# tmkhang1999/TextMAE-Image-Compression

Hardware: AMD Instinct MI355X
Metric: images/sec encode+decode+rate, ViT-B 256×256 batch64, 1/2/4/8 MI355X (higher is better)
Workload: dtype bf16; 1 GPU; MCM forward eval: ids+ViT-B/16 enc (K=144 of 256 patches) + LIC hyperprior + EB/GC rates + ViT dec 512/8/16 + unpatchify; img_size=256, num_keep_patches=144, per_gpu_batch=64, global_batch=64, parallelism=replicas x1, hip_graph=True

## Files before the change

### include/tmae.h

```cpp
#ifndef TMAE_H
#define TMAE_H

#include <stdint.h>

#ifdef __cplusplus
extern "C" {
#endif

#define TMAE_ABI_VERSION 1

enum { TMAE_OK = 0, TMAE_EINVAL = 1, TMAE_EHIP = 2 };
enum { TMAE_F32 = 0, TMAE_BF16 = 1 };
enum { TMAE_ACT_NONE = 0, TMAE_ACT_GELU = 1, TMAE_ACT_RELU = 2  };

const char* tmae_last_error_string(void);
int tmae_abi_version(void);

int tmae_ids_shuffle(const float* scores, int64_t* ids_shuffle, int64_t* ids_restore, int n, int L, int K,
                     int sum_lanes, void* stream);


int tmae_layernorm_fwd(const float* x, const float* gamma, const float* beta, void* y, int rows, int D,
                       int row_group, int group_stride, int row_offset, float eps, int out_dtype, void* stream);

// ... 245 lines not shown
                 int dh, float scale, int dtype, void* stream);
int tmae_patch_gather(const float* imgs, const int64_t* ids_shuffle, void* out, int n, int C, int H, int W, int patch,
                      int L, int keep, int dtype, void* stream);

typedef struct tmae_wgrad_args {
  const void* a; int lda; int a_G, a_Gs, a_off;
  const void* b; int ldb; int b_G, b_Gs, b_off;
  int b_conv; const void* b2; int b_c1, b_ld2, b_H, b_W, b_stride, b_Cin;
  int M, N, K;
  float* work; long long work_elems;
  float* out; long long o_base, o_sm, o_sc, o_st; int o_cp; int accumulate;
  float* bias_out; int bias_accumulate;
  int slot_div;
  int nb; long long s_a, s_b, s_b2, s_out, s_bias;
} tmae_wgrad_args;
int tmae_wgrad(const tmae_wgrad_args* args, int dtype, void* stream);
long long tmae_wgrad_workspace(int M, int N, int K, int dtype);
long long tmae_wgrad_workspace_nb(int M, int N, int K, int dtype, int slot_div, int nb);

int tmae_dgrad_linear(const void* dy, int ldy, int row_group, int group_stride, int row_offset, const void* wt, int M,
                      int N, int K, void* out, int out_f32, int ldo, const void* pre, int ldp, float* acc32, int ld32,
                      int dtype, void* stream);

typedef struct tmae_conv_dgrad_args {
  const void* dy; int ldy;
  int n, H, W, stride, cout, cin;
  const void* wd;
  void* out; int out_f32, ldo; const void* pre; int ldp;
  float* acc[3]; int ld_acc[3]; int lim[3];
  int nb; long long s_dy, s_wd, s_out, s_pre;
} tmae_conv_dgrad_args;
int tmae_conv_dgrad(const tmae_conv_dgrad_args* args, int dtype, void* stream);

int tmae_relayout(const float* src, void* dst, int dst_dtype, int d0, int d1, int d2, int d3, long long s0, long long s1,
                  long long s2, long long s3, void* stream);
int tmae_relayout_multi(const long long* table, int ntensors, long long nchunks, void* stream);

int tmae_colsum(const void* x, int x_dtype, int ld, int rows, int C, int row_group, int group_stride, int row_offset,
                float* work, long long work_elems, float* out, int accumulate, void* stream);

int tmae_layernorm_bwd(const float* x, const float* gamma, const float* dy, const float* dres, float* dx32, void* dxop,
                       int op_dtype, int rows, int D, int row_group, int group_stride, int row_offset, float eps,
                       float* work, long long work_elems, float* dgamma, float* dbeta, float* dres_colsum, int accumulate,
                       void* stream);

int tmae_unshuffle_bwd(const void* dy, int dy_f32, int ldy, const void* pre, int ldp, void* out, int n, int H, int W,
                       int C4, int dtype, void* stream);
int tmae_gelu_bwd(const void* dy, int dy_f32, const void* pre, void* out, long long total, int dtype, void* stream);
int tmae_lrp_bwd(const float* g32, int ld32, const float* g32b, int ld32b, const void* g16, int ld16, const float* t,
                 int ldt, void* dt, int lddt, float* gsum, int ldgs, int rows, int C, int dtype, void* stream);
int tmae_copy2d(const void* src, int lds, void* dst, int ldd, int rows, int cols, int esz, void* stream);
int tmae_gc_bwd(const float* y, int ldy, int yoff, const float* mu, const float* sigma, int ld_ms, const float* noise,
                int Mtot, const float* glik, const float* gyp, int ldg, float* dy, int lddy, void* dmu, void* dsigma,
                int ldd, int n, int HW, int sw, int dtype, void* stream);
int tmae_eb_bwd(const tmae_eb_params* params, const float* z, const float* noise, const float* glik,
                const float* gzhat, float* dz, int n, int C, int HW, const tmae_eb_params* grads, int accumulate,
                void* stream);
int tmae_eb_aux_bwd(const tmae_eb_params* params, const float* target, const float* gout, float* dquantiles, int C,
                    int accumulate, void* stream);
int tmae_bpp_bwd(const float* lik, const float* gout, float* dlik, long long n, double num_pixels, void* stream);
int tmae_patchify(const float* imgs, void* out, int n, int C, int H, int W, int patch, int dtype, void* stream);
int tmae_unpatchify(const float* tokens, float* imgs, int n, int C, int H, int W, int patch, void* stream);
int tmae_decoder_embed_bwd_gather(const float* dec_grad, const int64_t* ids_shuffle, void* tok_grad, int n, int ntok,
                                  int L, int D, int dtype, float* mask_part, float* dmask, int accumulate,
                                  void* stream);
int tmae_add(const float* a, const float* b, float* out, long long n, void* stream);

int tmae_adam(float* p, const float* g, float* m, float* v, long long n, float lr, float beta1, float beta2, float eps,
              float weight_decay, int step, const float* clip, void* stream);
int tmae_adam_multi(const long long* table, int ntensors, long long nchunks, float lr, float beta1, float beta2,
                    float eps, float weight_decay, const float* clip, void* stream);
int tmae_grad_norm(const float* g, long long n, double* work, float max_norm, float* out, void* stream);
int tmae_scale(float* g, long long n, const float* scale, void* stream);

int tmae_distortion_fwd(const float* x, const float* y, int P, int H, int W, float* hwork, float* dmaps, double* part,
                        float* out, void* stream);
int tmae_distortion_bwd(const float* x, const float* y, int P, int H, int W, const float* dmaps, float* vwork,
                        const float* gout, float* gx, void* stream);

int tmae_gemm_plan(int M, int N, int K, int batch, int dtype, char* out, int len);

int tmae_gemm_force_tile(int index);

int tmae_mha_plan(int T, int dh, int dtype, int backward, char* out, int len);

int tmae_mha_force_stream(int on);

#ifdef __cplusplus
}
#endif

#endif
```

### textmae-image-compression_amd/_lib.py

```python
from __future__ import annotations

import ctypes
import os

PKG_DIR = os.path.dirname(os.path.abspath(__file__))
LIB_PATH = os.environ.get("TMAE_LIB") or os.path.join(PKG_DIR, "lib", "libtmae.so")

TMAE_F32, TMAE_BF16 = 0, 1
ACT_NONE, ACT_GELU, ACT_RELU = 0, 1, 2

P, I, F = ctypes.c_void_p, ctypes.c_int, ctypes.c_float


LL = ctypes.c_longlong


class ConvArgs(ctypes.Structure):
    _fields_ = [
        ("x1", P), ("c1", I), ("ld1", I), ("x1_s1", LL), ("x1_s2", LL),
        ("x2", P), ("c2", I), ("ld2", I), ("x2_s1", LL), ("x2_s2", LL),
        ("n", I), ("H", I), ("W", I), ("stride", I),
        ("w", P), ("w_s1", LL), ("w_s2", LL),
        ("bias", P), ("b_s1", LL), ("b_s2", LL),
        ("cout", I), ("act", I), ("pixel_shuffle", I),
# ... 28 lines not shown
        ("wd", P),
        ("out", P), ("out_f32", I), ("ldo", I), ("pre", P), ("ldp", I),
        ("acc", P * 3), ("ld_acc", I * 3), ("lim", I * 3),
        ("nb", I), ("s_dy", LL), ("s_wd", LL), ("s_out", LL), ("s_pre", LL),
    ]


LSTK_MAXL = 5


class LicStackArgs(ctypes.Structure):
    _fields_ = [
        ("n", I), ("G", I), ("nb1", I), ("nb2", I), ("nlayers", I),
        ("x1", P), ("c1", I), ("ld1", I), ("x1_s", LL * 2),
        ("x2", P), ("c2", I), ("ld2", I), ("x2_s", LL * 2),
        ("w", P * LSTK_MAXL), ("w_s", (LL * 2) * LSTK_MAXL),
        ("bias", P * LSTK_MAXL), ("b_s", (LL * 2) * LSTK_MAXL),
        ("cout", I * LSTK_MAXL),
        ("addend", P), ("ld_add", I), ("a_s", LL * 2),
        ("y", P), ("y_f32", I), ("ldy", I), ("y_s", LL * 2),
        ("lrp_src", P), ("ld_src", I), ("src_s", LL * 2),
        ("y2", P), ("ldy2", I), ("y2_s", LL * 2),
        ("flags", I),
        ("cn", I), ("cw", P * LSTK_MAXL), ("cb", P * LSTK_MAXL), ("ccout", I * LSTK_MAXL),
        ("cx1", P), ("cc1", I), ("cld1", I),
        ("yv", P), ("ldyv", I),
        ("cadd", P), ("cld_add", I),
        ("csrc", P), ("cld_src", I),
        ("cy", P), ("cldy", I),
        ("cy2", P), ("cldy2", I),
        ("cs_x1", LL), ("cs_yv", LL), ("cs_src", LL), ("cs_add", LL), ("cs_y", LL), ("cs_y2", LL),
        ("cs_w", LL * LSTK_MAXL), ("cs_b", LL * LSTK_MAXL),
        ("sv_pre", P * LSTK_MAXL), ("sv_act", P * LSTK_MAXL), ("sv_s", (LL * 2) * LSTK_MAXL),
        ("sv_t", P), ("sv_t_s", LL * 2),
        ("csv_pre", P * LSTK_MAXL), ("csv_act", P * LSTK_MAXL), ("cs_sv", LL * LSTK_MAXL),
        ("csv_t", P), ("cs_t", LL),
        ("racc", P * 3), ("rld", I * 3), ("rlim", I * 3), ("rs", LL * 3),
    ]


class LicLatentArgs(ctypes.Structure):
    _fields_ = [
        ("n", I), ("G", I), ("cin", I), ("nb", I),
        ("x", P * 4), ("ldx", I),
        ("w", P), ("nfr", I), ("blk", LL),
        ("f_off", I * 4), ("f_lo", I), ("f_hi", I),
        ("y", P), ("ldy", I),
        ("y_s", LL * 4), ("bias", P * 4), ("act", I), ("y_bf16", I),
    ]


class EBParams(ctypes.Structure):
    _fields_ = [("matrix", ctypes.c_void_p * 5), ("bias", ctypes.c_void_p * 5), ("factor", ctypes.c_void_p * 4),
                ("quantiles", ctypes.c_void_p)]


SIGNATURES = {
    "tmae_abi_version": [],
    "tmae_ids_shuffle": [P, P, P, I, I, I, I, P],
    "tmae_layernorm_fwd": [P, P, P, P, I, I, I, I, I, F, I, P],
    "tmae_linear_fwd": [P, I, I, I, I, I, P, P, P, I, I, P, I, I, I, I, I, I, P],
    "tmae_linear_residual_fwd": [P, I, P, P, P, I, I, I, I, I, P],
    "tmae_patch_embed_fwd": [P, P, P, P, P, P, I, I, I, I, I, I, I, I, I, P],
    "tmae_patch_embed_gathered": [P, P, P, P, P, P, I, I, I, I, I, I, P],
    "tmae_cls_rows": [P, P, P, I, I, I, P],
    "tmae_mha_fwd": [P, P, I, I, I, I, F, I, P],
    "tmae_qkv_attn_fwd": [P, P, P, P, I, I, I, I, F, I, P],
    "tmae_decoder_embed_fwd": [P, I, P, P, P, P, P, I, I, I, I, I, I, P],
    "tmae_mask_rows": [P, P, P, P, I, I, I, I, P],
    "tmae_decoder_pred_fwd": [P, P, P, P, I, I, I, I, I, I, I, I, P],
    "tmae_decoder_pred_cp_fwd": [P, P, P, P, I, I, I, I, I, I, I, I, P],
    "tmae_conv3x3": [ctypes.POINTER(ConvArgs), I, P],
    "tmae_lic_stack": [ctypes.POINTER(LicStackArgs), P],
    "tmae_lic_latent": [ctypes.POINTER(LicLatentArgs), P],
    "tmae_gc_slices_fwd": [P, I, I, P, P, LL, I, P, P, I, P, I, I, P, I, I, I, I, I, P],
    "tmae_eb_likelihood_fwd": [P, ctypes.POINTER(EBParams), P, P, P, I, P, I, I, I, P],
    "tmae_eb_aux_loss": [ctypes.POINTER(EBParams), P, P, P, I, P],
    "tmae_gc_likelihood_fwd": [P, P, P, P, P, P, I, F, P],
    "tmae_nhwc_to_nchw": [P, I, P, I, I, I, P],
    "tmae_crop_normalize_u8": [P, I, I, I, P, I, I, ctypes.POINTER(F), ctypes.POINTER(F), P, P],
    "tmae_bpp_sum": [P, LL, P, LL, P, P, ctypes.c_double, P],
    "tmae_gemm_plan": [I, I, I, I, I, ctypes.c_char_p, I],
    "tmae_mha_plan": [I, I, I, I, ctypes.c_char_p, I],
    "tmae_mae_masking": [P, P, P, P, I, I, I, P],
    "tmae_mae_loss": [P, P, P, I, I, I, I, I, I, I, P, P, P],
    "tmae_mae_loss_bwd": [P, P, P, I, I, I, I, I, I, I, P, P, P, I, P],
    "tmae_gc_slices_code": [P, I, I, P, P, LL, I, P, I, P, I, I, P, I, I, I, I, I, P, P, P, I, P],
    "tmae_gc_indexes": [P, LL, I, I, I, I, I, P, I, F, P, P],
    "tmae_gc_dequantize": [P, P, LL, I, I, I, I, I, I, P, I, I, P, I, P],
    "tmae_gc_pmf": [P, P, I, I, P, P, P],
    "tmae_eb_pmf": [ctypes.POINTER(EBParams), P, P, I, I, P, P, P],
    "tmae_eb_symbols": [P, ctypes.POINTER(EBParams), P, I, I, I, P, P],
    "tmae_eb_dequantize": [P, ctypes.POINTER(EBParams), P, I, I, I, P, I, P],
    "tmae_invert_permutation": [P, P, I, I, P],
    "tmae_pmf_to_quantized_cdf": [P, I, I, P],
    "tmae_rans_encoder_create": [ctypes.POINTER(ctypes.c_void_p)],
    "tmae_rans_encode_with_indexes": [P, P, P, LL, P, I, P, P, I],
    "tmae_rans_encoder_flush": [P, ctypes.POINTER(ctypes.c_longlong)],
    "tmae_rans_encoder_take": [P, P, LL],
    "tmae_rans_encoder_destroy": [P],
    "tmae_rans_decoder_create": [P, LL, ctypes.POINTER(ctypes.c_void_p)],
    "tmae_rans_decode_with_indexes": [P, P, LL, P, I, P, P, I, P],
    "tmae_rans_decoder_destroy": [P],
    "tmae_rans_encode_streams": [P, LL, LL, P, LL, LL, I, I, I, P, I, P, P, I, P, LL, P, P, P],
    "tmae_rans_pack_streams": [P, LL, P, I, P, LL, P, P, P],
    "tmae_rans_decode_streams": [P, LL, P, P, P, LL, LL, P, LL, LL, I, I, I, I, P, I, P, P, I, P, P, P, I, P],
    "tmae_rans_encode_lanes": [P, LL, LL, P, LL, LL, I, I, I, P, I, P, P, I, P, LL, P, P, I, P],
    "tmae_rans_decode_lanes": [P, LL, P, P, P, LL, LL, P, LL, LL, I, I, I, I, P, I, P, P, I, P, P, P, I, I, P],
    "tmae_huffman_build": [P, LL, P, P, P, I, ctypes.POINTER(I)],
    "tmae_huffman_encode": [P, LL, P, P, P, I, P, LL, ctypes.POINTER(LL)],
    "tmae_huffman_decode": [ctypes.c_char_p, LL, P, P, P, I, P, LL, ctypes.POINTER(LL)],
    "tmae_image_metrics": [P, P, I, I, I, I, P, LL, P, P],
    "tmae_image_scores": [P, I, I, I, I, I, P, LL, P, P],
    "tmae_vgg_prep": [P, I, I, I, I, I, P, I, P],
    "tmae_vgg_prep_bwd": [P, I, I, I, I, I, P, I, P],
    "tmae_maxpool2": [P, I, I, I, I, P, P, I, P],
    "tmae_maxpool2_bwd": [P, P, I, I, I, I, P, P, I, P],
    "tmae_relu_mask": [P, P, LL, I, P],
    "tmae_mse": [P, P, LL, P, P, I, I, P],
    "tmae_mse_bwd": [P, P, LL, P, P, I, P],
    "tmae_linear_fwd_pre": [P, I, I, I, I, I, P, P, P, I, I, P, I, I, I, I, I, I, P],
    "tmae_linear_residual_out": [P, I, P, P, P, P, I, I, I, I, I, P],
    "tmae_mha_fwd_lse": [P, P, P, I, I, I, I, F, I, P],
    "tmae_mha_bwd": [P, P, P, P, P, I, I, I, I, F, I, P],
    "tmae_patch_gather": [P, P, P, I, I, I, I, I, I, I, I, P],
    "tmae_wgrad": [ctypes.POINTER(WgradArgs), I, P],
    "tmae_dgrad_linear": [P, I, I, I, I, P, I, I, I, P, I, I, P, I, P, I, I, P],
    "tmae_conv_dgrad": [ctypes.POINTER(ConvDgradArgs), I, P],
    "tmae_relayout": [P, P, I, I, I, I, I, LL, LL, LL, LL, P],
    "tmae_relayout_multi": [P, I, LL, P],
    "tmae_colsum": [P, I, I, I, I, I, I, I, P, LL, P, I, P],
    "tmae_layernorm_bwd": [P, P, P, P, P, P, I, I, I, I, I, I, F, P, LL, P, P, P, I, P],
    "tmae_unshuffle_bwd": [P, I, I, P, I, P, I, I, I, I, I, P],
    "tmae_gelu_bwd": [P, I, P, P, LL, I, P],
    "tmae_lrp_bwd": [P, I, P, I, P, I, P, I, P, I, P, I, I, I, I, P],
    "tmae_copy2d": [P, I, P, I, I, I, I, P],
    "tmae_gc_bwd": [P, I, I, P, P, I, P, I, P, P, I, P, I, P, P, I, I, I, I, I, P],
    "tmae_eb_bwd": [ctypes.POINTER(EBParams), P, P, P, P, P, I, I, I, ctypes.POINTER(EBParams), I, P],
    "tmae_eb_aux_bwd": [ctypes.POINTER(EBParams), P, P, P, I, I, P],
    "tmae_bpp_bwd": [P, P, P, LL, ctypes.c_double, P],
    "tmae_patchify": [P, P, I, I, I, I, I, I, P],
    "tmae_unpatchify": [P, P, I, I, I, I, I, P],
    "tmae_decoder_embed_bwd_gather": [P, P, P, I, I, I, I, I, P, P, I, P],
    "tmae_add": [P, P, P, LL, P],
    "tmae_adam": [P, P, P, P, LL, F, F, F, F, F, I, P, P],
    "tmae_adam_multi": [P, I, LL, F, F, F, F, F, P, P],
    "tmae_grad_norm": [P, LL, P, F, P, P],
    "tmae_scale": [P, LL, P, P],
    "tmae_distortion_fwd": [P, P, I, I, I, P, P, P, P, P],
    "tmae_distortion_bwd": [P, P, I, I, I, P, P, P, P, P],
}

VALUE_FUNCS = {"tmae_wgrad_workspace": ([I, I, I, I], ctypes.c_longlong),
               "tmae_wgrad_workspace_nb": ([I, I, I, I, I, I], ctypes.c_longlong),
               "tmae_metrics_workspace": ([I, I, I, I], ctypes.c_longlong),
               "tmae_image_scores_workspace": ([I, I, I, I], ctypes.c_longlong),
               "tmae_qkv_attn_supported": ([I, I, I], ctypes.c_int),
               "tmae_gemm_force_tile": ([I], ctypes.c_int),
               "tmae_mha_force_stream": ([I], ctypes.c_int),
               "tmae_rans_stream_cap_words": ([LL], ctypes.c_longlong)}

_lib = None


class TmaeError(RuntimeError):
    pass
# ... 36 lines not shown
```

### textmae-image-compression_amd/csrc/gemm.hip

```cpp
#include <stdio.h>

#include "gemm_core.h"


template <typename T> struct DenseSrcF32 {
  const float* p;
  int ld, rows, K, G, Gs, off;
  struct Row { const float* ptr; };
  __device__ void batch(int, int) {}
  __device__ Row row(int m) const {
    if (m >= rows) return {nullptr};
    return {p + (size_t)((m / G) * Gs + off + (m % G)) * ld};
  }
  __device__ uint4 load(const Row& r, int kt, int c) const {
    const int k = kt * 8 * Elt<T>::EPC + c * Elt<T>::EPC;
    if (!r.ptr || k >= K) return uint4{0, 0, 0, 0};
    return load_chunk_from_f32<T>(r.ptr + k);
  }
};

struct EpiResidual {
  float* out;
  int ldo;
  const float* bias;
  __device__ void batch(int, int) {}
  __device__ void operator()(int m, int n, f32x4 v) const {
    float* p = out + (size_t)m * ldo + n;
    if (bias) v += load4f(bias + n);
    store4(p, load4f(p) + v);
  }
  f32x4 pb0, pb1;
  __device__ void prefetch(int n, int N) {
    pb0 = pb1 = f32x4{0.f, 0.f, 0.f, 0.f};
    if (bias && n + 8 <= N) load8f(bias + n, pb0, pb1);
  }
  struct Pre { f32x4 r0, r1; };
  __device__ Pre fetch(int m, int n) const {
    Pre p;
    load8f(out + (size_t)m * ldo + n, p.r0, p.r1);
    return p;
  }
  __device__ void wide(int m, int n, f32x4 lo, f32x4 hi, const Pre& p) const {
    store8(out + (size_t)m * ldo + n, p.r0 + (lo + pb0), p.r1 + (hi + pb1));
  }};

struct EpiPatchEmbed {
  float* tok;
  const float* bias;
  const float* pos;
  const int64_t* ids;
  int L, keep, D;
  __device__ void batch(int, int) {}
  __device__ void operator()(int m, int n, f32x4 v) const {
    const int b = m / keep, k = m - b * keep;
    const int p = (int)ids[(size_t)b * L + k];
    v += load4f(bias + n);
    v += load4f(pos + (size_t)(1 + p) * D + n);
    store4(tok + ((size_t)b * (keep + 1) + 1 + k) * D + n, v);
  }
  f32x4 pb0, pb1;
  __device__ void prefetch(int n, int N) {
    pb0 = pb1 = f32x4{0.f, 0.f, 0.f, 0.f};
    if (n + 8 <= N) load8f(bias + n, pb0, pb1);
  }
  __device__ void wide(int m, int n, f32x4 lo, f32x4 hi) const {
    const int b = m / keep, k = m - b * keep;
    const int p = (int)ids[(size_t)b * L + k];
    f32x4 p0, p1;
    load8f(pos + (size_t)(1 + p) * D + n, p0, p1);
    store8(tok + ((size_t)b * (keep + 1) + 1 + k) * D + n, lo + pb0 + p0, hi + pb1 + p1);
  }
};

struct EpiDecoderEmbed {
  float* out;
  const float* bias;
  const float* pos;
  const int64_t* ids;
  int L, ntok, D;
  __device__ void batch(int, int) {}
  __device__ void operator()(int m, int n, f32x4 v) const {
    const int b = m / ntok, k = m - b * ntok;
    const int row = (k == 0) ? 0 : 1 + (int)ids[(size_t)b * L + (k - 1)];
    v += load4f(bias + n);
// ... 209 lines not shown
                                    int L, int keep, int dtype, void* stream) {
  if (dtype == TMAE_BF16)
    return patch_t<bf16>(imgs, ids_shuffle, w, bias, pos, tokens, n, C, H, W, patch, D, L, keep, (hipStream_t)stream);
  return patch_t<float>(imgs, ids_shuffle, w, bias, pos, tokens, n, C, H, W, patch, D, L, keep, (hipStream_t)stream);
}

template <typename T>
static int patch_gathered_t(const void* patches, const int64_t* ids, const void* w, const float* bias, const float* pos,
                            float* tok, int n, int Kw, int D, int L, int keep, hipStream_t st) {
  TMAE_REQUIRE(check_k<T>(Kw) && D % 4 == 0, "tmae_patch_embed_gathered: K=%d / dim %d unsupported", Kw, D);
  DenseSrc<T> xs{(const T*)patches, Kw, n * keep, Kw, 1 << 30, 0, 0, BStride{0, 0}};
  return launch_gemm<true, T>("tmae_patch_embed_gathered", (const T*)w, 0, 0, D, Kw, xs,
                              EpiPatchEmbed{tok, bias, pos, ids, L, keep, D}, n * keep, 1, 1, st);
}

extern "C" int tmae_patch_embed_gathered(const void* patches, const int64_t* ids_shuffle, const void* w,
                                         const float* bias, const float* pos, float* tokens, int n, int Kw, int D,
                                         int L, int keep, int dtype, void* stream) {
  if (dtype == TMAE_BF16)
    return patch_gathered_t<bf16>(patches, ids_shuffle, w, bias, pos, tokens, n, Kw, D, L, keep, (hipStream_t)stream);
  return patch_gathered_t<float>(patches, ids_shuffle, w, bias, pos, tokens, n, Kw, D, L, keep, (hipStream_t)stream);
}

template <typename T>
static int dec_embed_t(const void* x, int x_f32, const void* w, const float* bias, const float* pos,
                       const int64_t* ids, float* out, int n, int ntok, int L, int Din, int D, hipStream_t st) {
  TMAE_REQUIRE(check_k<T>(Din) && D % 4 == 0, "tmae_decoder_embed_fwd: bad dims %d -> %d", Din, D);
  TMAE_REQUIRE(ntok >= 1 && ntok <= L + 1, "tmae_decoder_embed_fwd: ntok=%d, L=%d", ntok, L);
  EpiDecoderEmbed epi{out, bias, pos, ids, L, ntok, D};
  if (x_f32 && sizeof(T) != 4) {
    DenseSrcF32<T> xs{(const float*)x, Din, n * ntok, Din, 1 << 30, 0, 0};
    return launch_gemm<false, T>("tmae_decoder_embed_fwd", (const T*)w, 0, 0, D, Din, xs, epi, n * ntok, 1, 1, st);
  }
  DenseSrc<T> xs{(const T*)x, Din, n * ntok, Din, 1 << 30, 0, 0, BStride{0, 0}};
  return launch_gemm<true, T>("tmae_decoder_embed_fwd", (const T*)w, 0, 0, D, Din, xs, epi, n * ntok, 1, 1, st);
}

extern "C" int tmae_decoder_embed_fwd(const void* x, int x_f32, const void* w, const float* bias, const float* pos,
                                      const int64_t* ids_shuffle, float* out, int n, int ntok, int L, int Din, int D,
                                      int dtype, void* stream) {
  if (dtype == TMAE_BF16)
    return dec_embed_t<bf16>(x, x_f32, w, bias, pos, ids_shuffle, out, n, ntok, L, Din, D, (hipStream_t)stream);
  return dec_embed_t<float>(x, 1, w, bias, pos, ids_shuffle, out, n, ntok, L, Din, D, (hipStream_t)stream);
}

template <typename T>
static int dec_pred_t(const void* x, const void* w, const float* bias, float* imgs, int n, int L, int Din, int C,
                      int H, int W, int P, hipStream_t st) {
  const int G = W / P;
  const int N = P * P * C;
  TMAE_REQUIRE(H == W && G * G == L && check_k<T>(Din) && N % 4 == 0, "tmae_decoder_pred_fwd: bad geometry");
  DenseSrc<T> xs{(const T*)x, Din, n * L, Din, 1 << 30, 0, 0, BStride{0, 0}};
  return launch_gemm<true, T>("tmae_decoder_pred_fwd", (const T*)w, 0, 0, N, Din, xs,
                              EpiUnpatchify{imgs, bias, L, G, P, C, H, W}, n * L, 1, 1, st);
}

template <typename T>
static int dec_pred_cp_t(const void* x, const void* w, const float* bias, float* imgs, int n, int L, int Din, int C,
                         int H, int W, int P, hipStream_t st) {
  const int G = W / P;
  const int N = P * P * C;
  TMAE_REQUIRE(H == W && G * G == L && check_k<T>(Din) && P % 8 == 0 && W % 4 == 0,
               "tmae_decoder_pred_cp_fwd: bad geometry (patch must be a multiple of 8)");
  DenseSrc<T> xs{(const T*)x, Din, n * L, Din, 1 << 30, 0, 0, BStride{0, 0}};
  return launch_gemm<true, T>("tmae_decoder_pred_cp_fwd", (const T*)w, 0, 0, N, Din, xs,
                              EpiUnpatchifyCP{imgs, bias, L, G, P, C, H, W}, n * L, 1, 1, st);
}

extern "C" int tmae_decoder_pred_cp_fwd(const void* x, const void* w, const float* bias, float* imgs, int n, int L,
                                        int Din, int C, int H, int W, int patch, int dtype, void* stream) {
  if (dtype == TMAE_BF16) return dec_pred_cp_t<bf16>(x, w, bias, imgs, n, L, Din, C, H, W, patch, (hipStream_t)stream);
  return dec_pred_cp_t<float>(x, w, bias, imgs, n, L, Din, C, H, W, patch, (hipStream_t)stream);
}

extern "C" int tmae_decoder_pred_fwd(const void* x, const void* w, const float* bias, float* imgs, int n, int L,
                                     int Din, int C, int H, int W, int patch, int dtype, void* stream) {
  if (dtype == TMAE_BF16) return dec_pred_t<bf16>(x, w, bias, imgs, n, L, Din, C, H, W, patch, (hipStream_t)stream);
  return dec_pred_t<float>(x, w, bias, imgs, n, L, Din, C, H, W, patch, (hipStream_t)stream);
}

extern "C" int tmae_gemm_plan(int M, int N, int K, int batch, int dtype, char* out, int len) {
  TMAE_REQUIRE(out != nullptr && len > 0 && M >= 0 && N >= 0 && K >= 0 && batch >= 1, "tmae_gemm_plan: bad arguments");
  const bool bf = dtype == TMAE_BF16;
  const TileChoice tc = choose_tile(M, N, K, batch, bf);
  const int stages = gemm_ring_stages(bf ? 2 : 4, tc.bn, tc.bm, tc.nw, K);
  snprintf(out, len, "glds<%s,%dx%d,%dw,BK%dx%d>", bf ? "bf16" : "f32", tc.bn, tc.bm, tc.nw, bf ? 64 : 32, stages);
  return TMAE_OK;
}

int g_tmae_gemm_force_tile = -1;
extern "C" int tmae_gemm_force_tile(int index) {
  const int prev = g_tmae_gemm_force_tile;
  g_tmae_gemm_force_tile = (index >= 0 && index < kNumTiles) ? index : -1;
  return prev;
}
```

### textmae-image-compression_amd/csrc/gemm_core.h

```cpp
#pragma once

#include <stdlib.h>

#include <algorithm>
#include <cmath>
#include <type_traits>
#include <utility>

#include "common.h"

typedef __attribute__((address_space(3))) void lds_void_t;
typedef __attribute__((address_space(1))) const void gbl_void_t;

static __device__ __attribute__((aligned(64))) uint4 g_tmae_zero_page[4] = {};

__device__ __forceinline__ void glds16(const void* gsrc, unsigned lds_addr) {
  unsigned keep;
  lds_addr = __builtin_amdgcn_readfirstlane(lds_addr);
  asm volatile("s_mov_b32 %0, m0\n\ts_mov_b32 m0, %2\n\ts_nop 0\n\tglobal_load_lds_dwordx4 %1, off\n\ts_mov_b32 m0, %0"
               : "=&s"(keep)
               : "v"(gsrc), "s"(lds_addr)
               : "memory");
}

// ... 544 lines not shown
#pragma unroll
    for (int j = 0; j < TM; ++j) asm volatile("" ::"v"(acc[i][j]));
  return;
#endif
  epilogue_any<TN, TM, WN>(epi, acc, reinterpret_cast<float*>(lds) + wave * EpiRegion<WN>::FLOATS,
                           tn * BN + wn * WN, tm * BM + wm * WM, lane, M, N);
  GEMM_TR(3);
#if TMAE_GEMM_TRACE
  asm volatile("s_waitcnt vmcnt(0)" ::: "memory");
  GEMM_TR(6);
#endif
}

template <typename T, int BN, int BM, int WGN, class WS, class XS, class EPI>
__global__ void __launch_bounds__(256, 2)
gemm_reg_kernel(WS ws, XS xs, EPI epi, int M, int N, int K, int n2) {
  constexpr int BKE = 8 * Elt<T>::EPC;
  constexpr int WGM = 4 / WGN;
  constexpr int WN = BN / WGN, WM = BM / WGM;
  constexpr int TN = WN / 16, TM = WM / 16;
  constexpr int WCH = BN / 32, XCH = BM / 32;
  constexpr int ROWS = BN + BM;
  __shared__ __attribute__((aligned(16))) uint4 lds[2 * ROWS * 8];

  const int b1 = blockIdx.y / n2, b2 = blockIdx.y - (blockIdx.y / n2) * n2;
  ws.batch(b1, b2);
  xs.batch(b1, b2);
  epi.batch(b1, b2);
  const int tid = threadIdx.x, lane = tid & 63, wave = tid >> 6;
  const int wn = wave % WGN, wm = wave / WGN;
  int tn, tm;
  tile_order(xcd_remap(blockIdx.x, gridDim.x), (N + BN - 1) / BN, (M + BM - 1) / BM, tn, tm);
  const int n0 = tn * BN, m0 = tm * BM;
  const int ch = tid & 7, r0 = tid >> 3;

  typename WS::Row wrow[WCH];
  typename XS::Row xrow[XCH];
#pragma unroll
  for (int p = 0; p < WCH; ++p) wrow[p] = ws.row(n0 + r0 + 32 * p);
#pragma unroll
  for (int p = 0; p < XCH; ++p) xrow[p] = xs.row(m0 + r0 + 32 * p);
  uint4 wreg[WCH], xreg[XCH];
  auto gload = [&](int kt) {
#pragma unroll
    for (int p = 0; p < WCH; ++p) wreg[p] = ws.load(wrow[p], kt, ch);
#pragma unroll
    for (int p = 0; p < XCH; ++p) xreg[p] = xs.load(xrow[p], kt, ch);
  };
  auto swrite = [&](int buf) {
    uint4* base = lds + buf * ROWS * 8;
#pragma unroll
    for (int p = 0; p < WCH; ++p) {
      const int r = r0 + 32 * p;
      base[r * 8 + (ch ^ ((r >> 1) & 7))] = wreg[p];
    }
#pragma unroll
    for (int p = 0; p < XCH; ++p) {
      const int r = r0 + 32 * p;
      base[(BN + r) * 8 + (ch ^ ((r >> 1) & 7))] = xreg[p];
    }
  };
  f32x4 acc[TN][TM];
#pragma unroll
  for (int i = 0; i < TN; ++i)
#pragma unroll
    for (int j = 0; j < TM; ++j) acc[i][j] = f32x4{0.f, 0.f, 0.f, 0.f};
  const int nk = (K + BKE - 1) / BKE;
  if (nk > 0) {
    gload(0);
    swrite(0);
  }
  __syncthreads();
  for (int kt = 0; kt < nk; ++kt) {
    if (kt + 1 < nk) gload(kt + 1);
    mfma_tile<T, BN, WN, WM, TN, TM>(lds + (kt & 1) * ROWS * 8, wn, wm, lane, acc);
    if (kt + 1 < nk) swrite((kt + 1) & 1);
    __syncthreads();
  }
  static_assert(4 * EpiRegion<WN>::FLOATS * 4 <= 2 * ROWS * 128, "epilogue region exceeds the LDS ring");
  epilogue_any<TN, TM, WN>(epi, acc, reinterpret_cast<float*>(lds) + wave * EpiRegion<WN>::FLOATS, n0 + wn * WN,
                           m0 + wm * WM, lane, M, N);
}

struct TileChoice { int bn, bm, nw; };

static constexpr int kNumTiles = 9;
static constexpr int kTileCand[kNumTiles][3] = {{256, 256, 8}, {128, 128, 4}, {64, 128, 4}, {32, 128, 4}, {64, 64, 4},
                                                {32, 64, 4},   {256, 192, 8}, {128, 160, 4}, {128, 192, 4}};
static inline bool tile_bf16_only(int i) { return kTileCand[i][2] == 8 || i >= 7; }
extern int g_tmae_gemm_force_tile;
#ifndef TMAE_GEMM_TILE
#define TMAE_GEMM_TILE -1
#endif
static inline TileChoice choose_tile(int M, int N, int K, int batch, bool allow_big) {
  const double kf = 1.0 + 0.12 * std::log2(std::max(K, 768) / 768.0);
  const double eff[kNumTiles] = {1.10 * kf, 1.0, 0.86, 0.70, 0.72, 0.55, 1.08 * kf, 1.22, 1.25};
  const int forced = g_tmae_gemm_force_tile >= 0 ? g_tmae_gemm_force_tile : TMAE_GEMM_TILE;
  if (forced >= 0 && forced < kNumTiles && (allow_big || !tile_bf16_only(forced)))
    return TileChoice{kTileCand[forced][0], kTileCand[forced][1], kTileCand[forced][2]};
  double best = -1.0;
  TileChoice tc{128, 128, 4};
  for (int i = 0; i < kNumTiles; ++i) {
    if (tile_bf16_only(i) && !allow_big) continue;
    const int bn = kTileCand[i][0], bm = kTileCand[i][1];
    const double tn = ceil_div(N, bn), tm = ceil_div(M, bm);
    const double useful = ((double)N / (tn * bn)) * ((double)M / (tm * bm));
    const double wgs = tn * tm * batch;
    const double slots = kTileCand[i][2] == 8 ? 256.0 : 512.0;
    const double quant = wgs / (std::ceil(wgs / slots) * slots);
    const double score = useful * quant * eff[i];
    if (score > best + 1e-9) { best = score; tc = TileChoice{bn, bm, kTileCand[i][2]}; }
  }
  return tc;
}

static constexpr int kGemmAnyK = 1 << 30;
static constexpr int gemm_ring_stages(int elt_bytes, int bn, int bm, int nw, int K) {
  const int dns = (bn + bm) * 128 * 4 <= 80 * 1024 ? 4 : (bn + bm) * 128 * 3 <= 80 * 1024 ? 3 : 2;
  const bool deep_ok = elt_bytes == 2 && nw == 4 && dns > 2;
  const int bke = 128 / elt_bytes;
  return deep_ok && (K + bke - 1) / bke >= 8 ? dns : 2;
}

template <bool GLDS, typename T, int BN, int BM, int WGN, int NW, class WS, class XS, class EPI>
static int launch_one(const char* name, const WS& ws, const XS& xs, const EPI& epi, int M, int N, int K, int n1,
                      int n2, hipStream_t st) {
  const int tiles = ceil_div(N, BN) * ceil_div(M, BM);
  if (tiles == 0 || n1 * n2 == 0) return TMAE_OK;
  if constexpr (GLDS) {
    constexpr int DNS = gemm_ring_stages(sizeof(T), BN, BM, NW, kGemmAnyK);
    if constexpr (DNS > 2) {
      if (gemm_ring_stages(sizeof(T), BN, BM, NW, K) == DNS) {
        hipLaunchKernelGGL((gemm_glds_kernel<T, BN, BM, WGN, NW, WS, XS, EPI, DNS>), dim3(tiles, n1 * n2),
                           dim3(64 * NW), 0, st, ws, xs, epi, M, N, K, n2);
        TMAE_LAUNCH_CHECK(name);
      }
    }
    hipLaunchKernelGGL((gemm_glds_kernel<T, BN, BM, WGN, NW, WS, XS, EPI>), dim3(tiles, n1 * n2), dim3(64 * NW), 0,
                       st, ws, xs, epi, M, N, K, n2);
  } else {
    hipLaunchKernelGGL((gemm_reg_kernel<T, BN, BM, WGN, WS, XS, EPI>), dim3(tiles, n1 * n2), dim3(256), 0, st, ws, xs,
                       epi, M, N, K, n2);
  }
  TMAE_LAUNCH_CHECK(name);
}

template <bool GLDS, typename T, class XS, class EPI>
static int launch_gemm(const char* name, const T* w, long long ws1, long long ws2, int N, int K, const XS& xs,
                       const EPI& epi, int M, int n1 = 1, int n2 = 1, hipStream_t st = 0) {
  DenseSrc<T> ws{w, K, N, K, 1 << 30, 0, 0, BStride{ws1, ws2}};
  const TileChoice tc = choose_tile(M, N, K, n1 * n2, GLDS && sizeof(T) == 2);
  if constexpr (GLDS && sizeof(T) == 2) {
    if (tc.nw == 8 && tc.bm == 192) return launch_one<GLDS, T, 256, 192, 2, 8>(name, ws, xs, epi, M, N, K, n1, n2, st);
    if (tc.nw == 4 && tc.bm == 160) return launch_one<GLDS, T, 128, 160, 2, 4>(name, ws, xs, epi, M, N, K, n1, n2, st);
    if (tc.nw == 4 && tc.bm == 192) return launch_one<GLDS, T, 128, 192, 2, 4>(name, ws, xs, epi, M, N, K, n1, n2, st);
    if (tc.nw == 8) return launch_one<GLDS, T, 256, 256, 2, 8>(name, ws, xs, epi, M, N, K, n1, n2, st);
  }
  if (tc.bn == 128) return launch_one<GLDS, T, 128, 128, 2, 4>(name, ws, xs, epi, M, N, K, n1, n2, st);
  if (tc.bn == 64 && tc.bm == 128) return launch_one<GLDS, T, 64, 128, 1, 4>(name, ws, xs, epi, M, N, K, n1, n2, st);
  if (tc.bn == 32 && tc.bm == 128) return launch_one<GLDS, T, 32, 128, 1, 4>(name, ws, xs, epi, M, N, K, n1, n2, st);
  if (tc.bn == 64) return launch_one<GLDS, T, 64, 64, 2, 4>(name, ws, xs, epi, M, N, K, n1, n2, st);
  return launch_one<GLDS, T, 32, 64, 1, 4>(name, ws, xs, epi, M, N, K, n1, n2, st);
}

template <typename OT, int ACT> struct EpiStore {
  static constexpr bool kDirectBf16 = sizeof(OT) == 2;
  static constexpr int kAct = ACT;
  OT* out;
  int ldo;
  const float* bias;
  const float* addend;
  int ld_add;
  float* out32;
  int ld32;
  OT* pre;
  int ldp;
  BStride so, sb, sa, s32, sp;
  __device__ void batch(int b1, int b2) {
    out += so.at(b1, b2);
    if (bias) bias += sb.at(b1, b2);
    if (addend) addend += sa.at(b1, b2);
    if (out32) out32 += s32.at(b1, b2);
    if (pre) pre += sp.at(b1, b2);
  }
  __device__ void operator()(int m, int n, f32x4 v) const {
    if (bias) v += load4f(bias + n);
    if (addend) v += load4f(addend + (size_t)m * ld_add + n);
    if (pre) store4(pre + (size_t)m * ldp + n, v);
    if (ACT == TMAE_ACT_GELU) {
#pragma unroll
      for (int j = 0; j < 4; ++j) v[j] = gelu_for<OT>(v[j]);
    }
    if (ACT == TMAE_ACT_RELU) {
#pragma unroll
      for (int j = 0; j < 4; ++j) v[j] = fmaxf(v[j], 0.0f);
    }
    store4(out + (size_t)m * ldo + n, v);
    if (out32) store4(out32 + (size_t)m * ld32 + n, v);
  }
  __device__ bool direct_ok(int N) const {
    return !addend && !pre && !out32 && (N & 7) == 0 && (ldo & 7) == 0 && ((uintptr_t)out & 15) == 0;
  }
  f32x4 pb0, pb1;
  __device__ void prefetch(int n, int N) {
    pb0 = pb1 = f32x4{0.f, 0.f, 0.f, 0.f};
    if (bias && n + 8 <= N) load8f(bias + n, pb0, pb1);
  }
  struct Pre { f32x4 a0, a1; };
  __device__ Pre fetch(int m, int n) const {
    Pre p;
    if (addend) load8f(addend + (size_t)m * ld_add + n, p.a0, p.a1);
    return p;
  }
  __device__ void wide(int m, int n, f32x4 lo, f32x4 hi, const Pre& p) const {
    lo += pb0; hi += pb1;
    if (addend) { lo += p.a0; hi += p.a1; }
    if (pre) store8(pre + (size_t)m * ldp + n, lo, hi);
    if (ACT == TMAE_ACT_GELU) {
      if constexpr (sizeof(OT) == 2) {
        gelu8_bf16out(lo, hi);
      } else {
#pragma unroll
        for (int j = 0; j < 4; ++j) { lo[j] = gelu_for<OT>(lo[j]); hi[j] = gelu_for<OT>(hi[j]); }
      }
    }
    if (ACT == TMAE_ACT_RELU) {
#pragma unroll
      for (int j = 0; j < 4; ++j) { lo[j] = fmaxf(lo[j], 0.0f); hi[j] = fmaxf(hi[j], 0.0f); }
    }
    store8(out + (size_t)m * ldo + n, lo, hi);
    if (out32) store8(out32 + (size_t)m * ld32 + n, lo, hi);
  }};

template <typename OT, int ACT>
// ... 8 lines not shown
```

### textmae-image-compression_amd/ops.py

```python
from __future__ import annotations

import contextlib
import ctypes
import os

import torch

from . import _lib
from ._lib import ACT_GELU, ACT_NONE, TMAE_BF16, TMAE_F32, ConvArgs, EBParams, LicStackArgs

__all__ = [
    "ids_shuffle", "layernorm", "linear", "linear_residual", "patch_embed", "cls_rows", "mha", "decoder_embed",
    "mask_rows", "decoder_pred", "conv3x3", "lic_stack", "pack_lic_stack_weight", "lic_stack_fits", "gc_slices", "eb_likelihood", "eb_aux_loss",
    "gc_likelihood", "nhwc_to_nchw", "bpp", "gemm_plan", "force_gemm_tile", "GEMM_TILES", "mha_plan", "mha_force_stream", "dtype_code", "gc_slices_code", "gc_indexes",
    "gc_dequantize", "gc_pmf", "eb_pmf", "eb_symbols", "eb_dequantize", "invert_permutation", "mae_masking",
    "rans_stream_cap_words", "rans_encode_streams", "rans_pack_streams", "rans_decode_streams",
    "rans_encode_lanes", "rans_decode_lanes",
    "mae_loss", "TMAE_F32", "TMAE_BF16", "ACT_NONE", "ACT_GELU",
]


def _stream():
    return torch.cuda.current_stream().cuda_stream


def _p(t):
    if t is None or isinstance(t, int):
        return t
    return t.data_ptr()


def _need(t: torch.Tensor, dtype=None, name="tensor"):
    if not t.is_cuda:
        raise ValueError(f"{name} must be a device (HIP) tensor")
    if dtype is not None and t.dtype != dtype:
        raise ValueError(f"{name} must be {dtype}, got {t.dtype}")
    if not t.is_contiguous():
        raise ValueError(f"{name} must be contiguous")
    return t


def dtype_code(dt: torch.dtype) -> int:
    if dt == torch.float32:
        return TMAE_F32
    if dt == torch.bfloat16:
        return TMAE_BF16
    raise ValueError(f"unsupported compute dtype {dt}")


def gemm_plan(M: int, N: int, K: int, dtype: torch.dtype, batch: int = 1) -> str:
    buf = ctypes.create_string_buffer(96)
    _lib.call("tmae_gemm_plan", M, N, K, batch, dtype_code(dtype), buf, len(buf))
    return buf.value.decode()


GEMM_TILES = ((256, 256), (128, 128), (64, 128), (32, 128), (64, 64), (32, 64), (256, 192), (128, 160), (128, 192))


@contextlib.contextmanager
def force_gemm_tile(index: int):
    if not -1 <= index < len(GEMM_TILES):
        raise ValueError(f"force_gemm_tile: index {index} outside -1..{len(GEMM_TILES) - 1}")
    prev = _lib.value("tmae_gemm_force_tile", index)
    try:
        yield
    finally:
        _lib.value("tmae_gemm_force_tile", prev)


def mha_plan(T: int, dh: int, dtype: torch.dtype, backward: bool = False) -> str:
    buf = ctypes.create_string_buffer(96)
    _lib.call("tmae_mha_plan", T, dh, dtype_code(dtype), int(bool(backward)), buf, len(buf))
    return buf.value.decode()


@contextlib.contextmanager
def mha_force_stream(on: bool = True):
    prev = _lib.value("tmae_mha_force_stream", int(bool(on)))
    try:
        yield
    finally:
        _lib.value("tmae_mha_force_stream", prev)


def ids_shuffle(scores: torch.Tensor, keep: int, sum_lanes: int = 8):
    s = _need(scores.float().contiguous(), name="total_scores")
    n, L = s.shape
    shuf = torch.empty((n, L), dtype=torch.int64, device=s.device)
    rest = torch.empty_like(shuf)
    _lib.call("tmae_ids_shuffle", s.data_ptr(), shuf.data_ptr(), rest.data_ptr(), n, L, keep, sum_lanes, _stream())
    return shuf, rest


def layernorm(x, weight, bias, eps, out_dtype, rows=None, row_group=None, group_stride=0, row_offset=0, out=None):
    _need(x, torch.float32, "x")
    D = x.shape[-1]
    rows = x.numel() // D if rows is None else rows
    row_group = rows if row_group is None else row_group
    if out is None:
        out = torch.empty((rows, D), dtype=out_dtype, device=x.device)
    _lib.call("tmae_layernorm_fwd", x.data_ptr(), weight.data_ptr(), bias.data_ptr(), out.data_ptr(), rows, D,
              max(row_group, 1), group_stride, row_offset, float(eps), dtype_code(out.dtype), _stream())
    return out


def linear(x, w, b, dtype, act=ACT_NONE, out=None, out_dtype=None, M=None, ldx=None, row_group=None, group_stride=0,
           row_offset=0, out32=None):
    N, K = w.shape
    M = x.numel() // x.shape[-1] if M is None else M
    ldx = x.shape[-1] if ldx is None else ldx
    out_dtype = out_dtype or dtype
    if out is None:
        out = torch.empty((M, N), dtype=out_dtype, device=x.device)
    code = dtype_code(dtype)
    x_f32 = int(x.dtype == torch.float32)
    if code == TMAE_BF16 and not x_f32 and x.dtype != torch.bfloat16:
        raise ValueError("x must be f32 or bf16")
    if code == TMAE_F32 and (x.dtype != torch.float32 or out.dtype != torch.float32):
        raise ValueError("f32 path needs f32 tensors")
    _lib.call("tmae_linear_fwd", x.data_ptr(), x_f32, ldx, row_group or M, group_stride, row_offset, w.data_ptr(),
              _p(b), out.data_ptr(), int(out.dtype == torch.float32), out.shape[-1], _p(out32),
              0 if out32 is None else out32.shape[-1], M, N, K, act, code, _stream())
    return out


def linear_residual(x, w, b, resid, dtype):
    N, K = w.shape
    M = x.numel() // K
    _lib.call("tmae_linear_residual_fwd", x.data_ptr(), K, w.data_ptr(), _p(b), resid.data_ptr(), resid.shape[-1], M,
              N, K, dtype_code(dtype), _stream())
    return resid


_PATCH_WORK: dict = {}


def patch_embed(imgs, ids_shuffle, w, b, pos, tokens, keep, patch, dtype, patches=None):
    n, C, H, W = imgs.shape
    D = w.shape[0]
    L = ids_shuffle.shape[1]
    if w.dim() != 2 or w.shape[1] != -(-C * patch * patch // 8) * 8 or not w.is_contiguous():
        raise ValueError(f"patch_embed: weight {tuple(w.shape)} must be contiguous [D][C*P*P rounded up to 8]")
    Kw = w.shape[1]
    if patch % 8 == 0 or patches is not None:
        if patches is None:
            key = (imgs.device, dtype, n * keep * Kw)
            patches = _PATCH_WORK.get(key)
            if patches is None:
                patches = _PATCH_WORK[key] = torch.empty((n * keep, Kw), dtype=dtype, device=imgs.device)
            _lib.call("tmae_patch_gather", _need(imgs, torch.float32, "imgs").data_ptr(), ids_shuffle.data_ptr(),
# ... 496 lines not shown
```

Baseline: 10040 images/s.

## Add 128x144 GEMM tile and CU-aware occupancy-based tile selection

Adds a new 128x144 bf16 GEMM tile sized to the 144 kept-patch token count, so encoder GEMMs whose M is a multiple of 144 avoid padded-row waste. The tile picker now uses the queried CU count and an LDS-based residency estimate instead of fixed slot counts, and it weights the new tile by epilogue kind. This adds a template instantiation, and it risks picking different tiles for other shapes, some of which could run slower.

Result: no change. 10070 images/s, median of 6 (+0.2%).

```diff
diff --git a/include/tmae.h b/include/tmae.h
--- a/include/tmae.h
+++ b/include/tmae.h
@@ -351,6 +351,10 @@
 
 int tmae_gemm_force_tile(int index);
 
+int tmae_gemm_pick_tile(int M, int N, int K, int epi, int n_cu, unsigned tile_mask, int* out_tile, int* out_grid,
+                        int* out_resident);
+int tmae_gemm_tile_info(int tile, int M, int N, int K, int* out_bn, int* out_bm, int* out_grid, int* out_resident);
+
 int tmae_mha_plan(int T, int dh, int dtype, int backward, char* out, int len);
 
 int tmae_mha_force_stream(int on);
diff --git a/textmae-image-compression_amd/_lib.py b/textmae-image-compression_amd/_lib.py
--- a/textmae-image-compression_amd/_lib.py
+++ b/textmae-image-compression_amd/_lib.py
@@ -134,6 +134,8 @@
     "tmae_bpp_sum": [P, LL, P, LL, P, P, ctypes.c_double, P],
     "tmae_gemm_plan": [I, I, I, I, I, ctypes.c_char_p, I],
     "tmae_mha_plan": [I, I, I, I, ctypes.c_char_p, I],
+    "tmae_gemm_pick_tile": [I, I, I, I, I, ctypes.c_uint, ctypes.POINTER(I), ctypes.POINTER(I), ctypes.POINTER(I)],
+    "tmae_gemm_tile_info": [I, I, I, I, ctypes.POINTER(I), ctypes.POINTER(I), ctypes.POINTER(I), ctypes.POINTER(I)],
     "tmae_mae_masking": [P, P, P, P, I, I, I, P],
     "tmae_mae_loss": [P, P, P, I, I, I, I, I, I, I, P, P, P],
     "tmae_mae_loss_bwd": [P, P, P, I, I, I, I, I, I, I, P, P, P, I, P],
diff --git a/textmae-image-compression_amd/csrc/gemm.hip b/textmae-image-compression_amd/csrc/gemm.hip
--- a/textmae-image-compression_amd/csrc/gemm.hip
+++ b/textmae-image-compression_amd/csrc/gemm.hip
@@ -1,5 +1,8 @@
 #include <stdio.h>
 
+#ifndef TMAE_GEMM_ROUND_TILES
+#define TMAE_GEMM_ROUND_TILES 1
+#endif
 #include "gemm_core.h"
 
 
@@ -375,7 +378,7 @@
 extern "C" int tmae_gemm_plan(int M, int N, int K, int batch, int dtype, char* out, int len) {
   TMAE_REQUIRE(out != nullptr && len > 0 && M >= 0 && N >= 0 && K >= 0 && batch >= 1, "tmae_gemm_plan: bad arguments");
   const bool bf = dtype == TMAE_BF16;
-  const TileChoice tc = choose_tile(M, N, K, batch, bf);
+  const TileChoice tc = choose_tile(M, N, K, batch, bf, bf ? 2 : 4, bf && TMAE_GEMM_ROUND_TILES, kEpiBf16Store);
   const int stages = gemm_ring_stages(bf ? 2 : 4, tc.bn, tc.bm, tc.nw, K);
   snprintf(out, len, "glds<%s,%dx%d,%dw,BK%dx%d>", bf ? "bf16" : "f32", tc.bn, tc.bm, tc.nw, bf ? 64 : 32, stages);
   return TMAE_OK;
@@ -384,6 +387,41 @@
 int g_tmae_gemm_force_tile = -1;
 extern "C" int tmae_gemm_force_tile(int index) {
   const int prev = g_tmae_gemm_force_tile;
-  g_tmae_gemm_force_tile = (index >= 0 && index < kNumTiles) ? index : -1;
+  g_tmae_gemm_force_tile = (index >= 0 && index < kNumTiles) || index == -2 ? index : -1;
   return prev;
 }
+
+int tmae_gemm_device_cus() {
+  static const int cus = [] {
+    int dev = 0, n = 0;
+    if (hipGetDevice(&dev) != hipSuccess ||
+        hipDeviceGetAttribute(&n, hipDeviceAttributeMultiprocessorCount, dev) != hipSuccess || n <= 0)
+      return 256;
+    return n;
+  }();
+  return cus;
+}
+
+extern "C" int tmae_gemm_pick_tile(int M, int N, int K, int epi, int n_cu, unsigned tile_mask, int* out_tile,
+                                   int* out_grid, int* out_resident) {
+  TMAE_REQUIRE(M >= 0 && N >= 0 && K >= 0 && out_tile && out_grid && out_resident, "tmae_gemm_pick_tile: bad arguments");
+  const unsigned all = gemm_tile_mask(true, TMAE_GEMM_ROUND_TILES);
+  const unsigned mask = tile_mask ? tile_mask & all : all;
+  TMAE_REQUIRE(mask != 0, "tmae_gemm_pick_tile: tile_mask 0x%x offers no compiled tile", tile_mask);
+  const TilePick p = gemm_pick_tile(M, N, K, 1, 2, epi, mask, n_cu);
+  *out_tile = p.tile;
+  *out_grid = p.grid;
+  *out_resident = p.resident;
+  return TMAE_OK;
+}
+
+extern "C" int tmae_gemm_tile_info(int tile, int M, int N, int K, int* out_bn, int* out_bm, int* out_grid,
+                                   int* out_resident) {
+  TMAE_REQUIRE(tile >= 0 && tile < kNumTiles && M >= 0 && N >= 0 && K >= 0 && out_bn && out_bm && out_grid &&
+                   out_resident, "tmae_gemm_tile_info: bad arguments");
+  *out_bn = kTileCand[tile][0];
+  *out_bm = kTileCand[tile][1];
+  *out_grid = ceil_div(N, kTileCand[tile][0]) * ceil_div(M, kTileCand[tile][1]);
+  *out_resident = gemm_tile_resident(tile, 2, K);
+  return TMAE_OK;
+}
diff --git a/textmae-image-compression_amd/csrc/gemm_core.h b/textmae-image-compression_amd/csrc/gemm_core.h
--- a/textmae-image-compression_amd/csrc/gemm_core.h
+++ b/textmae-image-compression_amd/csrc/gemm_core.h
@@ -650,44 +650,81 @@
                            m0 + wm * WM, lane, M, N);
 }
 
-struct TileChoice { int bn, bm, nw; };
-
-static constexpr int kNumTiles = 9;
-static constexpr int kTileCand[kNumTiles][3] = {{256, 256, 8}, {128, 128, 4}, {64, 128, 4}, {32, 128, 4}, {64, 64, 4},
-                                                {32, 64, 4},   {256, 192, 8}, {128, 160, 4}, {128, 192, 4}};
-static inline bool tile_bf16_only(int i) { return kTileCand[i][2] == 8 || i >= 7; }
-extern int g_tmae_gemm_force_tile;
-#ifndef TMAE_GEMM_TILE
-#define TMAE_GEMM_TILE -1
-#endif
-static inline TileChoice choose_tile(int M, int N, int K, int batch, bool allow_big) {
-  const double kf = 1.0 + 0.12 * std::log2(std::max(K, 768) / 768.0);
-  const double eff[kNumTiles] = {1.10 * kf, 1.0, 0.86, 0.70, 0.72, 0.55, 1.08 * kf, 1.22, 1.25};
-  const int forced = g_tmae_gemm_force_tile >= 0 ? g_tmae_gemm_force_tile : TMAE_GEMM_TILE;
-  if (forced >= 0 && forced < kNumTiles && (allow_big || !tile_bf16_only(forced)))
-    return TileChoice{kTileCand[forced][0], kTileCand[forced][1], kTileCand[forced][2]};
-  double best = -1.0;
-  TileChoice tc{128, 128, 4};
-  for (int i = 0; i < kNumTiles; ++i) {
-    if (tile_bf16_only(i) && !allow_big) continue;
-    const int bn = kTileCand[i][0], bm = kTileCand[i][1];
-    const double tn = ceil_div(N, bn), tm = ceil_div(M, bm);
-    const double useful = ((double)N / (tn * bn)) * ((double)M / (tm * bm));
-    const double wgs = tn * tm * batch;
-    const double slots = kTileCand[i][2] == 8 ? 256.0 : 512.0;
-    const double quant = wgs / (std::ceil(wgs / slots) * slots);
-    const double score = useful * quant * eff[i];
-    if (score > best + 1e-9) { best = score; tc = TileChoice{bn, bm, kTileCand[i][2]}; }
-  }
-  return tc;
-}
-
 static constexpr int kGemmAnyK = 1 << 30;
 static constexpr int gemm_ring_stages(int elt_bytes, int bn, int bm, int nw, int K) {
   const int dns = (bn + bm) * 128 * 4 <= 80 * 1024 ? 4 : (bn + bm) * 128 * 3 <= 80 * 1024 ? 3 : 2;
   const bool deep_ok = elt_bytes == 2 && nw == 4 && dns > 2;
   const int bke = 128 / elt_bytes;
   return deep_ok && (K + bke - 1) / bke >= 8 ? dns : 2;
+}
+
+struct TileChoice { int bn, bm, nw; };
+
+static constexpr int kNumTiles = 10;
+static constexpr int kNumBaseTiles = 9;
+static constexpr int kTileCand[kNumTiles][3] = {{256, 256, 8}, {128, 128, 4}, {64, 128, 4}, {32, 128, 4}, {64, 64, 4},
+                                                {32, 64, 4},   {256, 192, 8}, {128, 160, 4}, {128, 192, 4},
+                                                {128, 144, 4}};
+static inline bool tile_bf16_only(int i) { return kTileCand[i][2] == 8 || i >= 7; }
+static inline bool tile_round(int i) { return i >= kNumBaseTiles; }
+extern int g_tmae_gemm_force_tile;
+int tmae_gemm_device_cus();
+#ifndef TMAE_GEMM_TILE
+#define TMAE_GEMM_TILE -1
+#endif
+#ifndef TMAE_GEMM_ROUND_TILES
+#define TMAE_GEMM_ROUND_TILES 0
+#endif
+
+enum { kEpiF32Store = 0, kEpiBf16Store = 1, kEpiF32Update = 2, kNumEpiKinds = 3 };
+static constexpr double kRoundEff[kNumEpiKinds] = {1.11, 1.09, 1.11};
+
+static constexpr int kLdsPerCu = 160 * 1024;
+static inline int gemm_tile_resident(int i, int elt_bytes, int K) {
+  const int bn = kTileCand[i][0], bm = kTileCand[i][1], nw = kTileCand[i][2];
+  const int lds = gemm_ring_stages(elt_bytes, bn, bm, nw, K) * (bn + bm) * 128;
+  return std::max(1, std::min(kLdsPerCu / lds, nw == 8 ? 1 : 2));
+}
+
+struct TilePick { int tile, grid, resident; };
+static inline unsigned gemm_tile_mask(bool allow_big, bool allow_round) {
+  unsigned m = 0;
+  for (int i = 0; i < kNumTiles; ++i)
+    if ((allow_big || !tile_bf16_only(i)) && (allow_round || !tile_round(i))) m |= 1u << i;
+  return m;
+}
+
+static inline TilePick gemm_pick_tile(int M, int N, int K, int batch, int elt_bytes, int epi, unsigned mask, int n_cu) {
+  const double kf = 1.0 + 0.12 * std::log2(std::max(K, 768) / 768.0);
+  const int ek = epi >= 0 && epi < kNumEpiKinds ? epi : 0;
+  const double eff[kNumTiles] = {1.10 * kf, 1.0, 0.86, 0.70, 0.72, 0.55, 1.08 * kf, 1.22, 1.25, kRoundEff[ek]};
+  n_cu = std::max(n_cu, 1);
+  double best = -1.0;
+  TilePick pick{1, 0, 2};
+  for (int i = 0; i < kNumTiles; ++i) {
+    if (!(mask >> i & 1)) continue;
+    const int bn = kTileCand[i][0], bm = kTileCand[i][1];
+    const double tn = ceil_div(N, bn), tm = ceil_div(M, bm);
+    const double wgs = tn * tm * batch;
+    const int resident = gemm_tile_resident(i, elt_bytes, K);
+    const double slots = (double)n_cu * resident;
+    if (wgs <= 0.0) continue;
+    const double useful = ((double)N / (tn * bn)) * ((double)M / (tm * bm));
+    const double fill = wgs / (std::ceil(wgs / slots) * slots);
+    const double score = useful * fill * eff[i];
+    if (score > best + 1e-9) { best = score; pick = TilePick{i, (int)std::min(wgs, 2147483647.0), resident}; }
+  }
+  return pick;
+}
+
+static inline TileChoice choose_tile(int M, int N, int K, int batch, bool allow_big, int elt_bytes = 2,
+                                     bool allow_round = false, int epi = 0) {
+  const unsigned mask = gemm_tile_mask(allow_big, allow_round && g_tmae_gemm_force_tile != -2);
+  const int forced = g_tmae_gemm_force_tile >= 0 ? g_tmae_gemm_force_tile : TMAE_GEMM_TILE;
+  if (forced >= 0 && forced < kNumTiles && (mask >> forced & 1))
+    return TileChoice{kTileCand[forced][0], kTileCand[forced][1], kTileCand[forced][2]};
+  const int t = gemm_pick_tile(M, N, K, batch, elt_bytes, epi, mask, tmae_gemm_device_cus()).tile;
+  return TileChoice{kTileCand[t][0], kTileCand[t][1], kTileCand[t][2]};
 }
 
 template <bool GLDS, typename T, int BN, int BM, int WGN, int NW, class WS, class XS, class EPI>
@@ -717,7 +754,13 @@
 static int launch_gemm(const char* name, const T* w, long long ws1, long long ws2, int N, int K, const XS& xs,
                        const EPI& epi, int M, int n1 = 1, int n2 = 1, hipStream_t st = 0) {
   DenseSrc<T> ws{w, K, N, K, 1 << 30, 0, 0, BStride{ws1, ws2}};
-  const TileChoice tc = choose_tile(M, N, K, n1 * n2, GLDS && sizeof(T) == 2);
+  constexpr bool kBig = GLDS && sizeof(T) == 2;
+  constexpr bool kRound = kBig && TMAE_GEMM_ROUND_TILES && std::is_same<XS, DenseSrc<T>>::value;
+  constexpr int kEpi = HasDirectBf16<EPI>::value ? kEpiBf16Store : HasFetch<EPI>::value ? kEpiF32Update : kEpiF32Store;
+  const TileChoice tc = choose_tile(M, N, K, n1 * n2, kBig, sizeof(T), kRound, kEpi);
+  if constexpr (kRound) {
+    if (tc.bm == 144) return launch_one<GLDS, T, 128, 144, 4, 4>(name, ws, xs, epi, M, N, K, n1, n2, st);
+  }
   if constexpr (GLDS && sizeof(T) == 2) {
     if (tc.nw == 8 && tc.bm == 192) return launch_one<GLDS, T, 256, 192, 2, 8>(name, ws, xs, epi, M, N, K, n1, n2, st);
     if (tc.nw == 4 && tc.bm == 160) return launch_one<GLDS, T, 128, 160, 2, 4>(name, ws, xs, epi, M, N, K, n1, n2, st);
diff --git a/textmae-image-compression_amd/ops.py b/textmae-image-compression_amd/ops.py
--- a/textmae-image-compression_amd/ops.py
+++ b/textmae-image-compression_amd/ops.py
@@ -12,7 +12,7 @@
 __all__ = [
     "ids_shuffle", "layernorm", "linear", "linear_residual", "patch_embed", "cls_rows", "mha", "decoder_embed",
     "mask_rows", "decoder_pred", "conv3x3", "lic_stack", "pack_lic_stack_weight", "lic_stack_fits", "gc_slices", "eb_likelihood", "eb_aux_loss",
-    "gc_likelihood", "nhwc_to_nchw", "bpp", "gemm_plan", "force_gemm_tile", "GEMM_TILES", "mha_plan", "mha_force_stream", "dtype_code", "gc_slices_code", "gc_indexes",
+    "gc_likelihood", "nhwc_to_nchw", "bpp", "gemm_plan", "force_gemm_tile", "GEMM_TILES", "GEMM_BASE_TILES", "GEMM_ROUND_TILES", "GEMM_ALL_TILES", "force_gemm_tile_id", "pick_gemm_tile", "gemm_tile_info", "mha_plan", "mha_force_stream", "dtype_code", "gc_slices_code", "gc_indexes",
     "gc_dequantize", "gc_pmf", "eb_pmf", "eb_symbols", "eb_dequantize", "invert_permutation", "mae_masking",
     "rans_stream_cap_words", "rans_encode_streams", "rans_pack_streams", "rans_decode_streams",
     "rans_encode_lanes", "rans_decode_lanes",
@@ -55,17 +55,41 @@
 
 
 GEMM_TILES = ((256, 256), (128, 128), (64, 128), (32, 128), (64, 64), (32, 64), (256, 192), (128, 160), (128, 192))
+GEMM_ROUND_TILES = ((128, 144),)
+GEMM_ALL_TILES = GEMM_TILES + GEMM_ROUND_TILES
+GEMM_BASE_TILES = len(GEMM_TILES)
+GEMM_EPI_F32, GEMM_EPI_BF16, GEMM_EPI_UPDATE = 0, 1, 2
+
+
+def pick_gemm_tile(M: int, N: int, K: int, epi: int = GEMM_EPI_BF16, n_cu: int = 256, tile_mask: int = 0):
+    t, g, r = ctypes.c_int(), ctypes.c_int(), ctypes.c_int()
+    _lib.call("tmae_gemm_pick_tile", M, N, K, epi, n_cu, tile_mask, ctypes.byref(t), ctypes.byref(g), ctypes.byref(r))
+    return t.value, g.value, r.value
+
+
+def gemm_tile_info(tile: int, M: int, N: int, K: int):
+    v = [ctypes.c_int() for _ in range(4)]
+    _lib.call("tmae_gemm_tile_info", tile, M, N, K, *[ctypes.byref(x) for x in v])
+    return tuple(x.value for x in v)
 
 
 @contextlib.contextmanager
-def force_gemm_tile(index: int):
-    if not -1 <= index < len(GEMM_TILES):
-        raise ValueError(f"force_gemm_tile: index {index} outside -1..{len(GEMM_TILES) - 1}")
+def force_gemm_tile_id(index: int):
+    if not -2 <= index < len(GEMM_ALL_TILES):
+        raise ValueError(f"force_gemm_tile_id: index {index} outside -2..{len(GEMM_ALL_TILES) - 1}")
     prev = _lib.value("tmae_gemm_force_tile", index)
     try:
         yield
     finally:
         _lib.value("tmae_gemm_force_tile", prev)
+
+
+@contextlib.contextmanager
+def force_gemm_tile(index: int):
+    if not -1 <= index < len(GEMM_TILES):
+        raise ValueError(f"force_gemm_tile: index {index} outside -1..{len(GEMM_TILES) - 1}")
+    with force_gemm_tile_id(index):
+        yield
 
 
 def mha_plan(T: int, dh: int, dtype: torch.dtype, backward: bool = False) -> str:
```
